# luigifcruz/radio-core

Hardware: AMD Instinct MI355X
Metric: IQ Msamples/s through Tuner+WBFM at 1024 channels (higher is better)
Workload: dtype f32

## Files before the change

### include/rcfm_tools.h

```cpp
#ifndef RCFM_TOOLS_H
#define RCFM_TOOLS_H

#include "rcfm.h"

#ifdef __cplusplus
extern "C" {
#endif

typedef struct rcfm_arena_s* rcfm_arena_t;

int rcfm_arena_create(size_t block_bytes, rcfm_arena_t* out);
int rcfm_arena_adopt(void* base, size_t bytes, rcfm_arena_t* out);
int rcfm_arena_bind(rcfm_arena_t arena);
int rcfm_arena_stats(rcfm_arena_t arena, size_t* reserved_bytes, size_t* used_bytes, size_t* live_pieces);
int rcfm_arena_destroy(rcfm_arena_t arena);


enum { RCFM_TUNER_OPT_NARROW_TILES = 1,
       RCFM_TUNER_OPT_ALIGNED_PLAN = 2 };
int rcfm_tuner_set_option(rcfm_tuner_t t, int option, int value);

enum { RCFM_OPT_LDS_CHAIN = 1, RCFM_OPT_FUSED_TILES = 2, RCFM_OPT_PHASE_LINK = 3, RCFM_OPT_PILOT_CHAIN = 6, RCFM_OPT_DECIM_TILE = 7,
       RCFM_OPT_LDS_DEEMPH = 8, RCFM_OPT_PILOT_BLOCKED = 9, RCFM_OPT_SSB_DIRECT = 11 };
int rcfm_demod_get_option(rcfm_demod_t d, int option, int* value);


typedef struct rcfm_fft_pass {
    int32_t L, nstages, radix[8];
    int64_t n_o1, n_o2, n_inner;
    int64_t in_o1, in_o2, in_i, in_l;
    int64_t out_o1, out_o2, out_i, out_k;
    int64_t tw_o1, tw_o2, tw_i;
    int32_t has_twiddle, load_along_l;
    int64_t in_t, out_t;
    int32_t flat_outer;
    int32_t reserved_;
} rcfm_fft_pass;
typedef struct rcfm_fft_plan {
// ... 23 lines not shown
```

### radio-core_amd/csrc/api_internal.h

```cpp
#pragma once

#include <algorithm>
#include <atomic>
#include <cstdlib>
#include <map>
#include <memory>
#include <mutex>
#include <string>
#include <vector>

#include "common.h"
#include "fft_engine.h"
#include "fft_plan.h"
#include "fused_passes.h"
#include "kernels.h"
#include "lds_chain.h"

#define TILE_CALL(narrow_tiles, fn, ...) ((narrow_tiles) ? ::rcfm::narrow::fn(__VA_ARGS__) : ::rcfm::fn(__VA_ARGS__))

namespace rcfm {

constexpr double kPi = 3.14159265358979323846;


// ... 132 lines not shown
    }();
    return v;
}

inline void require_channels(int first, int count, int n) {
    RC_REQUIRE(first >= 0 && count >= 0 && first + count <= n, RCFM_ERR_INDEX, "channel index out of range");
}

}


struct rcfm_tuner_s {
    rcfm::Arena* arena = rcfm::arena_enter_handle();
    ~rcfm_tuner_s() { rcfm::arena_leave_handle(arena); }
    int opt_narrow = rcfm::kNarrowDefault;
    int64_t n = 0;
    int nch = 0;
    std::vector<int64_t> roll;
    std::vector<int32_t> bw;
    rcfm::DeviceBuffer roll_dev;
    rcfm::DeviceBuffer base_dev;
    rcfm::DeviceBuffer bw_dev;
    rcfm::DeviceBuffer levels_part;
    rcfm::DeviceBuffer power_part_sum, power_part_max;
    rcfm::DeviceBuffer X;
    int64_t halo = 0;
    float2* ext = nullptr;
    bool ext_window = false;
    int ext_first = 0, ext_count = 0;
    float2* spectrum() { return (ext ? ext : X.as<float2>()) + halo; }
// ... 60 lines not shown
```

### radio-core_amd/csrc/demod.hip

```cpp

#include <cmath>
#include <cstring>

#include "api_internal.h"

using namespace rcfm;

struct rcfm_demod_s {
    Arena* arena = arena_enter_handle();
    ~rcfm_demod_s() {
        drop_graphs();
        if (cap_stream) (void)hipStreamDestroy(cap_stream);
        arena_leave_handle(arena);
    }
    int kind = 0, C = 0, B = 0, A = 0, ch = 1, chunk = 1;
    double tau = 75e-6;
    float taps_h[51];
    float zi_h[50];
    float pilot_h[41];
    float pilot_g_h[41];
    DeviceBuffer taps, pilot_g;
    struct StateBuf : DeviceBuffer {
        hipEvent_t ev = nullptr;
        bool armed = false, recorded = false;
// ... 18 lines not shown
    float side_tap = 0.23f;
    ResampleGeom geom;
    PlanCache r2c_B, c2c_inv_B, c2c_fwd_B, c2c_inv_A, c2r_A;
    std::unique_ptr<FftEngine> eng_B, eng_A;
    std::unique_ptr<FftEngine> eng_Ad;
    std::unique_ptr<FftEngine> eng_Bi;
    DeviceBuffer buf_Ti;
    bool opt_lds_chain = true;
    bool opt_pilot_chain = true;
    bool opt_decim_tile = true;
    bool opt_pilot_blocked = true;
    bool opt_phase_link = true;
    bool opt_lds_deemph = true;
    bool opt_ssb_direct = true;
    int opt_narrow = kNarrowDefault;
    bool opt_graph = false;
    struct GraphSlot {
        const void* iq;
        void* audio;
        const float* state;
        int first;
        hipGraphExec_t exec;
        uint64_t used;
    };
    std::vector<GraphSlot> graphs;
    GraphSlot last_call{nullptr, nullptr, nullptr, -1, nullptr, 0};
    hipStream_t cap_stream = nullptr;
    uint64_t graph_tick = 0;
    void drop_graphs() {
        for (auto& g : graphs) (void)hipGraphExecDestroy(g.exec);
// ... 641 lines not shown

int rcfm_demod_set_option(rcfm_demod_t d, int option, int value) {
    return guarded([&] {
        RC_REQUIRE(d, RCFM_ERR_ARG, "NULL handle");
        d->drop_graphs();
        switch (option) {
            case RCFM_OPT_GRAPH: d->opt_graph = value != 0; break;
            case RCFM_OPT_LDS_CHAIN: d->opt_lds_chain = value != 0; break;
            case RCFM_OPT_FUSED_TILES: d->opt_pilot_chain = d->opt_decim_tile = value != 0; break;
            case RCFM_OPT_PILOT_CHAIN: d->opt_pilot_chain = value != 0; break;
            case RCFM_OPT_DECIM_TILE: d->opt_decim_tile = value != 0; break;
            case RCFM_OPT_PILOT_BLOCKED: d->opt_pilot_blocked = value != 0; break;
            case RCFM_OPT_LDS_DEEMPH: d->opt_lds_deemph = value != 0; break;
            case RCFM_OPT_PHASE_LINK: d->opt_phase_link = value != 0; break;
            case RCFM_OPT_SSB_DIRECT: d->opt_ssb_direct = value != 0; break;
            case RCFM_OPT_NARROW_TILES:
                RC_REQUIRE(value >= 0 && value <= 2, RCFM_ERR_ARG, "narrow tiles: 0 never, 1 automatic, 2 always");
                d->opt_narrow = value;
                break;
            case RCFM_OPT_STATE_FENCE: {
                auto& b = *d->state_buf;
                if (value != 0 && b.ev == nullptr) RC_HIP(hipEventCreateWithFlags(&b.ev, hipEventDisableTiming));
                b.armed = value != 0;
                if (!b.armed) b.recorded = false;
                break;
            }
            default: RC_REQUIRE(false, RCFM_ERR_ARG, "unknown demodulator option");
        }
    });
}
// ... 1 lines not shown
int rcfm_demod_get_option(rcfm_demod_t d, int option, int* value) {
    return guarded([&] {
        RC_REQUIRE(d && value, RCFM_ERR_ARG, "NULL handle or output");
        switch (option) {
            case RCFM_OPT_LDS_CHAIN: *value = d->opt_lds_chain; break;
            case RCFM_OPT_FUSED_TILES: *value = d->opt_pilot_chain && d->opt_decim_tile; break;
            case RCFM_OPT_PILOT_CHAIN: *value = d->opt_pilot_chain; break;
            case RCFM_OPT_DECIM_TILE: *value = d->opt_decim_tile; break;
            case RCFM_OPT_PILOT_BLOCKED:
                *value = d->opt_pilot_blocked && d->opt_pilot_chain && d->pilot_blocked().valid() &&
                         fused_pilot_chain_applies(*d->eng_B, *d->eng_Bi, 2);
                break;
            case RCFM_OPT_LDS_DEEMPH: *value = d->opt_lds_deemph; break;
            case RCFM_OPT_PHASE_LINK: *value = d->opt_phase_link; break;
            case RCFM_OPT_SSB_DIRECT: *value = d->opt_ssb_direct; break;
            case RCFM_OPT_NARROW_TILES: *value = d->opt_narrow; break;
            case RCFM_OPT_STATE_FENCE: *value = d->state_buf->armed; break;
            case RCFM_OPT_GRAPH: *value = d->opt_graph ? 1 + (int)d->graphs.size() : 0; break;
            default: RC_REQUIRE(false, RCFM_ERR_ARG, "unknown demodulator option");
        }
    });
}

int rcfm_demod_get_taps(rcfm_demod_t d, float* deemph51_host, float* pilot41_host) {
    return guarded([&] {
        RC_REQUIRE(d, RCFM_ERR_ARG, "NULL handle");
        if (deemph51_host) std::memcpy(deemph51_host, d->taps_h, sizeof(d->taps_h));
        if (pilot41_host) std::memcpy(pilot41_host, d->pilot_h, sizeof(d->pilot_h));
    });
}
// ... 62 lines not shown
```

### radio-core_amd/csrc/fft_engine.h

```cpp
#pragma once

#include <cstdint>

#include "common.h"

namespace rcfm {

constexpr int kFftTileW = 16;
constexpr int kFftMaxStages = 8;
constexpr int kFftMaxPasses = 4;
constexpr int kFftMaxL = 512;
constexpr int kFftBigL = 640;

struct FftPass {
    int L;
    int nstages;
    int radix[kFftMaxStages];
    int64_t n_o1, n_o2, n_inner;
    int64_t in_o1, in_o2, in_i, in_l;
    int64_t out_o1, out_o2, out_i, out_k;
    int64_t tw_o1, tw_o2, tw_i;
    int has_twiddle;
    int load_along_l;
    int64_t in_t, out_t;
// ... 33 lines not shown
   public:
    explicit FftEngine(int64_t n);
    FftEngine(int64_t n, const int64_t* factors, int nfactors, int layout = -1);
    const FftPlanDesc& desc() const { return desc_; }
    bool has_blocked() const { return has_blk_; }
    const FftPlanDesc& desc_blocked() const { return has_blk_ ? desc_blk_ : desc_; }
    int npass() const { return desc_.npass; }
    int64_t tmp_stride() const { return desc_.tmp_stride; }
    void c2c(const float2* in, float2* out, float2* tmp, int batch, bool inverse, float scale,
             hipStream_t stream, const FftRowWindow* keep = nullptr, float2* tmp2 = nullptr) const;
    int64_t row_length() const { return desc_.pass[0].L; }
    FftPassDev pass_dev(int t, int64_t in_batch, int64_t out_batch, bool blocked = false) const;
    static size_t lds_bytes(int L);
    static dim3 grid(const FftPass& p, int batch);
    static int compute_units();

   private:
    void build_tables();
    void split_layouts();
    FftPlanDesc desc_;
    FftPlanDesc desc_blk_;
    bool has_blk_ = false;
    DeviceBuffer stage_tw_[kFftMaxPasses];
    DeviceBuffer pos_[kFftMaxPasses];
    DeviceBuffer coarse_;
};

}
```

### radio-core_amd/csrc/fft_kernel.h

```cpp
#pragma once

#include <hip/hip_runtime.h>

#include <cstdio>
#include <cstdlib>
#include <type_traits>

#include "fft_engine.h"
#include "tile_ns.h"

namespace rcfm {
RCFM_NS_OPEN
namespace fftk {

constexpr int W = RCFM_TILE_W;
constexpr int kLogW = W == 16 ? 4 : W == 8 ? 3 : 2;
static_assert((1 << kLogW) == W, "tile width: 4, 8 or 16 lines");
constexpr int kThreads = 256 * W / 16;

__device__ __forceinline__ float2 cmul(float2 a, float2 b) {
    typedef float v2f __attribute__((ext_vector_type(2)));
    v2f A, B, D;
    A.x = a.x; A.y = a.y; B.x = b.x; B.y = b.y;
    asm("v_pk_mul_f32 %0, %1, %2 op_sel:[0,0] op_sel_hi:[0,1]" : "=v"(D) : "v"(A), "v"(B));
// ... 506 lines not shown
__device__ __forceinline__ int last_stage_base(int g) {
    if constexpr (S == 2) {
        return g;
    } else if constexpr (S == 3) {
        constexpr int w1 = L / (R0 * RL);
        const int q1 = g / w1, q2 = g - q1 * w1;
        return q1 + R0 * q2;
    } else {
        constexpr int w1 = L / (R0 * RL), w2 = L / (R0 * R1 * RL);
        const int q1 = g / w1, r1 = g - q1 * w1;
        const int q2 = r1 / w2, q3 = r1 - q2 * w2;
        return q1 + R0 * (q2 + R1 * q3);
    }
}

template <int L, int R0, int R1, int R2, int R3, bool ROWS, int T, class LoadOp, class StoreOp>
__global__ __launch_bounds__(T, (big_tile_pair(L) ? 8 : triple_tile(L) ? 6 : T * 16 / W >= 512 ? 4 : 1)) void k_fft_tile(FftPassDev d, LoadOp load,
                                                                                          StoreOp store) {
    constexpr bool BIG = big_tile_pair(L) || triple_tile(L);
    constexpr int S = (R0 > 1) + (R1 > 1) + (R2 > 1) + (R3 > 1);
    static_assert(S >= 2 && R0 * R1 * R2 * R3 == L, "bad radix list");
    constexpr int RL = (S == 2) ? R1 : (S == 3) ? R2 : R3;
    constexpr int m0 = L / R0;
    constexpr int RG = T / W;
    constexpr int nit0 = (m0 + RG - 1) / RG;
    constexpr int nld = ROWS ? (L * W + T - 1) / T : nit0 * R0;
    __shared__ __attribute__((aligned(16))) float2 tile[L * (ROWS && !BIG ? kRowsPitch : W)];
    __shared__ __attribute__((aligned(16))) float2 tw_lds[BIG ? 1 : L];
    const float2* tw = BIG ? d.stage_tw : tw_lds;
    const FftPass& p = d.p;

    const int tid = threadIdx.x;
    const int w = tid & (W - 1), rg = tid >> kLogW;
    const VBlock vb = vblock_hw();
    LineId id;
    BlockPos bp = block_pos(vb);
    id.batch = bp.batch;
    unsigned o = vb.y;
    const unsigned n_o2 = (unsigned)p.n_o2;
    if (p.flat_outer) {
        const unsigned tiles_inner = ((unsigned)p.n_inner + W - 1) / W;
        o = bp.tile / tiles_inner;
        if (o >= (unsigned)(p.n_o1 * p.n_o2)) return;
        bp.tile -= o * tiles_inner;
    }
    id.o1 = n_o2 == 1 ? o : o / n_o2;
    id.o2 = n_o2 == 1 ? 0 : o - (unsigned)id.o1 * n_o2;
    const int i0 = (int)bp.tile * W;
    const int left = (int)p.n_inner - i0;
    const int wvalid = left < W ? left : W;
    const int64_t in_base = (int64_t)id.batch * d.in_batch + id.o1 * p.in_o1 + id.o2 * p.in_o2 +
                            (p.in_t ? (int64_t)(i0 >> 4) * p.in_t + (i0 & 15) : (int64_t)i0 * p.in_i);
    const int64_t out_base = (int64_t)id.batch * d.out_batch + id.o1 * p.out_o1 + id.o2 * p.out_o2 +
                             (p.out_t ? (int64_t)(i0 >> 4) * p.out_t + (i0 & 15) : (int64_t)i0);
    const unsigned in_l = (unsigned)p.in_l, in_i = (unsigned)p.in_i, out_k = (unsigned)p.out_k;

    constexpr int NF = fetch_count<LoadOp>::value;
    constexpr bool HZ = !ROWS && has_half_zones<LoadOp>::value && L % 2 == 0;
    auto zone = [](int q) -> int { return (q + 1) * m0 <= L / 2 ? 0 : (q * m0 > L / 2 ? 2 : 1); };
    float2 v[nld];
    float2 v2[NF >= 2 ? nld : 1];
    float v3[NF == 3 ? nld : 1];
    static_assert(NF <= 2 || !ROWS, "three-fetch load functors: strided passes only");
    if constexpr (ROWS) {
#pragma unroll
        for (int it = 0; it < nld; ++it) {
            int e = tid + T * it;
            if ((L * W) % T != 0) e = e < L * W ? e : 0;
            const int wl = e / L, l = e - wl * L;
            const int wc = wl < wvalid ? wl : 0;
            id.i = i0 + wc;
            v[it] = load.fetch(id, l, in_base, (unsigned)wc * in_i + (unsigned)l);
            if constexpr (NF == 2) v2[it] = load.fetch2(id, l, in_base, (unsigned)wc * in_i + (unsigned)l);
        }
    } else {
        const int wc = w < wvalid ? w : 0;
        id.i = i0 + wc;
#pragma unroll
        for (int it = 0; it < nit0; ++it) {
            int b = rg + RG * it;
            if (m0 % RG != 0) b = b < m0 ? b : 0;
#pragma unroll
            for (int q = 0; q < R0; ++q) {
                const int l = b + q * m0;
                if constexpr (HZ) {
                    const int z = zone(q);
                    if (z == 2) {
                        v[it * R0 + q] = make_float2(0.f, 0.f);
                        if constexpr (NF == 2) v2[it * R0 + q] = make_float2(0.f, 0.f);
                    } else {
                        v[it * R0 + q] = load.fetch(id, l, in_base, (unsigned)l * in_l + (unsigned)wc, z);
                        if constexpr (NF == 2)
// ... 24 lines not shown
            return g;
        } else if constexpr (S == 3) {
            constexpr int w1 = L / (R0 * RL);
            const int q1 = g / w1, q2 = g - q1 * w1;
            return q1 + R0 * q2;
        } else {
            constexpr int w1 = L / (R0 * RL), w2 = L / (R0 * R1 * RL);
            const int q1 = g / w1, r1 = g - q1 * w1;
            const int q2 = r1 / w2, q3 = r1 - q2 * w2;
            return q1 + R0 * (q2 + R1 * q3);
        }
    };
    constexpr bool AUX = has_aux<StoreOp>::value;
    float aux[AUX ? nitL * RL : 1];
    if constexpr (AUX) {
        const int wc = w < wvalid ? w : 0;
        id.i = i0 + wc;
#pragma unroll
        for (int it = 0; it < nitL; ++it) {
            int g = rg + RG * it;
            if (rowsL % RG != 0) g = g < rowsL ? g : 0;
            const int kb = kbase(g);
#pragma unroll
            for (int q = 0; q < RL; ++q) {
                const int k = kb + (L / RL) * q;
                aux[it * RL + q] = store.fetch_aux(id, k, out_base, (unsigned)k * out_k + (unsigned)wc);
            }
        }
    }

    if constexpr (ROWS) {
#pragma unroll
        for (int it = 0; it < nld; ++it) {
            const int e = tid + T * it;
            const int wl = e / L, l = e - wl * L;
            id.i = i0 + wl;
            float2 x;
            if constexpr (NF == 2) x = load.post(id, l, v[it], v2[it]);
            else x = load.post(id, l, v[it]);
            if ((L * W) % T == 0 || e < L * W) tile[lds_slot<true, !BIG>(l, wl)] = x;
        }
        __syncthreads();
        stage_lds<L, R0, L, true, RG, !BIG, BIG>(tile, tw, w, rg);
    } else {
        if constexpr (!BIG) __syncthreads();
        id.i = i0 + (w < wvalid ? w : 0);
#pragma unroll
        for (int it = 0; it < nit0; ++it) {
            const int b = rg + RG * it;
            if ((m0 % RG == 0) || b < m0) {
                float2* x = &v[it * R0];
#pragma unroll
                for (int q = 0; q < R0; ++q) {
                    if constexpr (HZ) {
                        if constexpr (NF == 2) {
                            if (zone(q) != 2) x[q] = load.post(id, b + q * m0, x[q], v2[it * R0 + q], zone(q));
                        } else {
                            if (zone(q) != 2) x[q] = load.post(id, b + q * m0, x[q], zone(q));
                        }
                    } else if constexpr (NF == 3) x[q] = load.post(id, b + q * m0, x[q], v2[it * R0 + q], v3[it * R0 + q]);
                    else if constexpr (NF == 2) x[q] = load.post(id, b + q * m0, x[q], v2[it * R0 + q]);
// ... 13 lines not shown
#pragma unroll
                for (int q = 0; q < R0; ++q) tile[lds_slot<false>(b + q * m0, w)] = x[dft_slot<R0>(q)];
            }
        }
    }
    __syncthreads();
    if constexpr (S >= 3) {
        stage_lds<L, R1, L / R0, ROWS, RG, !BIG, BIG>(tile, tw, w, rg);
        __syncthreads();
    }
    if constexpr (S >= 4) {
        stage_lds<L, R2, L / (R0 * R1), ROWS, RG, !BIG, BIG>(tile, tw, w, rg);
        __syncthreads();
    }

    const unsigned f = (unsigned)(id.o1 * p.tw_o1 + id.o2 * p.tw_o2 + (int64_t)(i0 + w) * p.tw_i);
    float2 D = make_float2(1.f, 0.f);
    constexpr bool PTW = !ROWS;
    if constexpr (PTW) D = big_twiddle(d, f * (unsigned)(L / RL));
    id.i = i0 + w;
    const bool lane_ok = w < wvalid;
#pragma unroll
    for (int it = 0; it < nitL; ++it) {
        const int g = rg + RG * it;
        if ((rowsL % RG == 0) || g < rowsL) {
            float2 x[RL];
#pragma unroll
            for (int q = 0; q < RL; ++q) x[q] = tile[lds_slot<ROWS, !BIG>(g * RL + q, w)];
            dft_p<RL>(x);
            const int kb = kbase(g);
            float2 Tw = make_float2(1.f, 0.f);
            if constexpr (PTW) Tw = big_twiddle(d, f * (unsigned)kb);
            if (lane_ok) {
#pragma unroll
                for (int q = 0; q < RL; ++q) {
                    const int k = kb + (L / RL) * q;
                    float2 y = x[dft_slot<RL>(q)];
                    if constexpr (PTW) {
                        y = cmul(y, Tw);
                        Tw = cmul(Tw, D);
                    }
                    if constexpr (AUX) store(id, k, out_base, (unsigned)k * out_k + (unsigned)w, y, aux[it * RL + q]);
                    else store(id, k, out_base, (unsigned)k * out_k + (unsigned)w, y);
                }
            }
        }
    }
}

template <class T, class = void>
struct mid_upper_rows_zero : std::false_type {};
template <class T>
struct mid_upper_rows_zero<T, std::void_t<decltype(T::kUpperRowsZero)>> : std::bool_constant<T::kUpperRowsZero> {};

template <int L, int R0, int R1, int R2, int R3, int T, class LoadOp, class MidOp, class StoreOp>
__global__ __launch_bounds__(T, (T * 16 / W >= 512 ? 4 : 1)) void k_fft_tile2(FftPassDev d1, FftPassDev d2, LoadOp load,
                                                                     MidOp mid, StoreOp store) {
    constexpr int S = (R0 > 1) + (R1 > 1) + (R2 > 1) + (R3 > 1);
    static_assert(S >= 2 && R0 * R1 * R2 * R3 == L, "bad radix list");
    constexpr int RL = (S == 2) ? R1 : (S == 3) ? R2 : R3;
    constexpr int RG = T / W;
    constexpr int nld = (L * W + T - 1) / T;
// ... 579 lines not shown
}

template <class T> struct is_plain_functor : std::false_type {};
template <bool S> struct is_plain_functor<LoadPlainT<S>> : std::true_type {};
template <bool S> struct is_plain_functor<StorePlainT<S>> : std::true_type {};
template <> struct is_plain_functor<StoreRowWindow> : std::true_type {};

enum PassKinds : int { kAnyPass = 0, kStridedOnly = 1, kRowsOnly = 2 };

template <int LEN, int A, int B, int C, int D, bool ROWS, class LoadOp, class StoreOp>
inline void launch_fft_tile_one(const FftPassDev& d, dim3 grid, const LoadOp& ld, const StoreOp& st, hipStream_t s) {
    constexpr int T = tile_threads(LEN);
    hipLaunchKernelGGL((k_fft_tile<LEN, A, B, C, D, ROWS, T, LoadOp, StoreOp>), grid, dim3(T), 0, s, d, ld, st);
}

template <int KIND = kAnyPass, class LoadOp, class StoreOp>
inline void launch_fft_pass(const FftPassDev& d, int batch, const LoadOp& ld, const StoreOp& st, hipStream_t s) {
    bool done = false;
    const bool rows = d.p.load_along_l != 0;
    RC_REQUIRE(!(KIND == kStridedOnly && rows) && !(KIND == kRowsOnly && !rows), RCFM_ERR_RUNTIME,
               "FFT functor used with the wrong pass kind");
    const bool shape_ok = (rows || d.p.in_i == 1) && d.p.out_i == 1 && ((d.p.has_twiddle != 0) == !rows) &&
                          d.p.n_o1 * d.p.n_o2 <= 65535 && batch <= 65535;
    if (shape_ok) {
        const unsigned tiles_inner = (unsigned)((d.p.n_inner + W - 1) / W), outer = (unsigned)(d.p.n_o1 * d.p.n_o2);
        const dim3 grid = d.p.flat_outer ? dim3((tiles_inner * outer + 7u) / 8u * 8u, 1, (unsigned)batch)
                                         : dim3(tiles_inner, outer, (unsigned)batch);
        switch (d.p.L) {
#define RCFM_CASE(LEN, A, B, C, D)                                                                            \
    case LEN:                                                                                                 \
        if (rows) {                                                                                           \
            if constexpr (KIND != kStridedOnly)                                                               \
                launch_fft_tile_one<LEN, A, B, C, D, true, LoadOp, StoreOp>(d, grid, ld, st, s);               \
        } else {                                                                                              \
            if constexpr (KIND != kRowsOnly)                                                                  \
                launch_fft_tile_one<LEN, A, B, C, D, false, LoadOp, StoreOp>(d, grid, ld, st, s);              \
        }                                                                                                     \
        done = true;                                                                                          \
// ... 113 lines not shown
```

### radio-core_amd/csrc/fused_passes.hip

```cpp
#include "fused_passes.h"
#include "device_math.h"

#include "fft_kernel.h"
#include "fft_decim_rt.h"
#include "kernels.h"

namespace rcfm {
RCFM_NS_OPEN

using fftk::LineId;
using fftk::kAnyPass;
using fftk::kRowsOnly;
using fftk::kStridedOnly;

namespace {


struct LoadTunerGatherFast {
    const float2* X;
    const int32_t* base;
    float two_pi_over_n, delta;
    float c0, c1, c2, c3;
    int B, nyq;
    int merge;
// ... 502 lines not shown
    fftk::StorePlainT<true> stl{z, (float)(1.0 / (double)n)};
    fftk::launch_fft_pass<kRowsOnly>(e.pass_dev(np - 1, e.tmp_stride(), n), count, ldl, stl, s);
}
void fused_real_pair_fft(const FftEngine& e, const float* x, float2* U, float2* tmp, int count, int keep,
                         hipStream_t s, bool from_phase, PhaseRows rows) {
    if (count <= 0) return;
    const int64_t n = e.desc().n;
    const int np = e.npass();
    const int pairs = (count + 1) / 2;
    fftk::StorePlainT<false> st0{tmp, 1.0f};
    if (from_phase) {
        const LoadPhaseStepPair ld = phase_pair_load(x, n, count, (int)e.desc().pass[0].in_l, rows);
        fftk::launch_fft_pass<kStridedOnly>(e.pass_dev(0, 0, e.tmp_stride()), pairs, ld, st0, s);
    } else {
        LoadRealPair ld{x, (int)n, count};
        fftk::launch_fft_pass<kStridedOnly>(e.pass_dev(0, 0, e.tmp_stride()), pairs, ld, st0, s);
    }
    middle_passes(e, 1, np - 2, tmp, pairs, s);
    fftk::LoadPlainT<false> ldl{tmp};
    if (keep >= 0 || keep == kKeepLowerHalf) {
        StorePruned stl{U, (int)n, keep};
        fftk::launch_fft_pass<kRowsOnly>(e.pass_dev(np - 1, e.tmp_stride(), n), pairs, ldl, stl, s);
    } else {
        fftk::StorePlainT<false> stl{U, 1.0f};
        fftk::launch_fft_pass<kRowsOnly>(e.pass_dev(np - 1, e.tmp_stride(), n), pairs, ldl, stl, s);
    }
}

void fused_hilbert_pair_ifft_mix(const FftEngine& e, const float2* U, const float* m, float2* u, float2* tmp,
                                 int count, hipStream_t s) {
    if (count <= 0) return;
// ... 75 lines not shown
    const FftPass& p0 = ef.desc().pass[0];
    if (p0.load_along_l || p0.in_i != 1 || p0.n_o1 != 1 || p0.n_o2 != 1 || (int64_t)p0.L * p0.in_l != ef.desc().n ||
        p0.n_inner != p0.in_l)
        return false;
    *rows = p0.L;
    *row_length = p0.in_l;
    return true;
}

void fused_pilot_chain_fft_first(const FftEngine& ef, const float* p, float2* tmp_f, int count, hipStream_t s,
                                 int64_t blk_stride, int blk16) {
    if (count <= 0) return;
    const int64_t n = ef.desc().n;
    LoadRealPair ld{p, (int)n, count, blk_stride, blk16};
    fftk::StorePlainT<false> st0{tmp_f, 1.0f};
    fftk::launch_fft_pass<kStridedOnly>(ef.pass_dev(0, 0, ef.tmp_stride()), (count + 1) / 2, ld, st0, s);
}

void fused_pilot_chain_mask_mix(const FftEngine& ef, const FftEngine& ei, const float* p, const float* m,
                                float2* tmp_f, float2* tmp_i, int count, hipStream_t s, int64_t blk_stride, int blk16) {
    if (count <= 0) return;
    const int64_t n = ef.desc().n;
    const int pairs = (count + 1) / 2;
    {
        const FftPassDev d1 = ef.pass_dev(1, ef.tmp_stride(), n);
        const FftPassDev d2 = ei.pass_dev(0, n, ei.tmp_stride());
        fftk::LoadPlainT<false> ld{tmp_f};
        fftk::StorePlainT<false> st{tmp_i, 1.0f};
        const float scale = (float)(1.0 / (double)n);
        bool ok;
        if (d1.p.L % 2 == 0 && (int64_t)d1.p.L * d1.p.out_k == n)
// ... 45 lines not shown
    WinAudioDecim win{wr, dc, scale, (int)A, ef.desc().pass[0].L, 0};
    fftk::StorePlainT<false> st{tmp_a, 1.0f};
    {
        const FftPassDev d1 = ef.pass_dev(1, ef.tmp_stride(), B), d2 = ea.pass_dev(0, A, ea.tmp_stride());
        RC_REQUIRE(fftk::launch_fft_tile2_decim(d1, d2, count, ld, win, st, s) || decim_rt(d1, d2, count, tmp_f, win, tmp_a, s),
                   RCFM_ERR_RUNTIME, "decimating two-transform kernel refused a pair it should accept");
    }
    fftk::LoadPlainT<false> ldl{tmp_a};
    fftk::StorePlainT<true> stl{out, 1.0f};
    FftPassDev last = ea.pass_dev(1, ea.tmp_stride(), A);
    if (out_pitch > 0) {
        RC_REQUIRE(out_pitch >= last.p.out_k && last.p.n_o1 * last.p.n_o2 == 1, RCFM_ERR_RUNTIME, "bad audio row pitch");
        last.out_batch = (A / last.p.out_k) * (int64_t)out_pitch;
        last.p.out_k = out_pitch;
    }
    fftk::launch_fft_pass<kRowsOnly>(last, count, ldl, stl, s);
}

struct StoreRealImagSplit {
    float* y;
    int n, count;
    __device__ __forceinline__ void operator()(const LineId& id, int, int64_t base, unsigned off, float2 v) const {
        const int64_t t = base + off - (int64_t)id.batch * n;
        const int c0 = 2 * id.batch;
        y[(int64_t)c0 * n + t] = v.y;
        if (c0 + 1 < count) y[(int64_t)(c0 + 1) * n + t] = v.x;
    }
};

void fused_real_pair_fft_first(const FftEngine& e, const float* x, float2* tmp, int count, bool from_phase,
                               hipStream_t s, PhaseRows rows) {
    if (count <= 0) return;
    const int64_t n = e.desc().n;
    const int pairs = (count + 1) / 2;
    fftk::StorePlainT<false> st0{tmp, 1.0f};
    if (from_phase) {
        const LoadPhaseStepPair ld = phase_pair_load(x, n, count, (int)e.desc().pass[0].in_l, rows);
        fftk::launch_fft_pass<kStridedOnly>(e.pass_dev(0, 0, e.tmp_stride()), pairs, ld, st0, s);
    } else {
        LoadRealPair ld{x, (int)n, count};
        fftk::launch_fft_pass<kStridedOnly>(e.pass_dev(0, 0, e.tmp_stride()), pairs, ld, st0, s);
    }
}

void fused_fft_decim_ifft_pairs(const FftEngine& ef, const FftEngine& ea, const float2* tmp_f, float* y,
                                float2* tmp_a, int count, const float* wr, float scale, float2* dc, hipStream_t s) {
    if (count <= 0) return;
    const int64_t B = ef.desc().n, A = ea.desc().n;
    const int pairs = (count + 1) / 2;
    fftk::LoadPlainT<false> ld{tmp_f};
    WinAudioDecim win{wr, dc, scale, (int)A, ef.desc().pass[0].L, count};
    fftk::StorePlainT<false> st{tmp_a, 1.0f};
    {
        const FftPassDev d1 = ef.pass_dev(1, ef.tmp_stride(), B), d2 = ea.pass_dev(0, A, ea.tmp_stride());
        RC_REQUIRE(fftk::launch_fft_tile2_decim(d1, d2, pairs, ld, win, st, s) || decim_rt(d1, d2, pairs, tmp_f, win, tmp_a, s),
                   RCFM_ERR_RUNTIME, "decimating two-transform kernel refused a pair it should accept");
// ... 143 lines not shown
```

### radio-core_amd/csrc/tuner.hip

```cpp

#include "api_internal.h"

using namespace rcfm;

bool rcfm_tuner_s::row_window(int first, int count, FftRowWindow* w, const FftEngine* eng) const {
    if (!eng) eng = forward_engine.get();
    if (!eng || count == 0) return false;
    const int64_t f0 = eng->row_length();
    const int64_t rows = n / f0;
    if (rows < 64) return false;
    std::vector<char> used((size_t)rows, 0);
    for (int c = first; c < first + count; ++c) {
        const int64_t centre = (n - roll[c]) % n, h = bw[c] / 2 + 2;
        const int64_t r0 = (centre - h) / f0 - ((centre - h) < 0 ? 1 : 0), r1 = (centre + h) / f0;
        for (int64_t r = r0; r <= r1; ++r) used[(size_t)(((r % rows) + rows) % rows)] = 1;
    }
    int64_t best_len = 0, best_start = 0, run = 0;
    for (int64_t i = 0; i < 2 * rows; ++i) {
        if (!used[(size_t)(i % rows)]) {
            ++run;
            if (run > best_len && run <= rows) {
                best_len = run;
                best_start = i - run + 1;
            }
// ... 59 lines not shown
    bool ok = halo > 0 && count > 0;
    if (ok) {
        bin_window(first, count, fb, nb);
        ok = *nb < n && *fb >= halo && *fb + *nb <= n - halo;
    }
    RC_REQUIRE(ok, RCFM_ERR_SIZE,
               "these channels' bins wrap around the ends of the spectrum (or are all of it): no window storage");
}

rcfm_tuner_s::Band& rcfm_tuner_s::band(int32_t b) {
    auto it = bands.find(b);
    if (it == bands.end()) {
        auto nb = std::make_unique<Band>();
        nb->geom.build(n, b, 0.5 , true);
        FftPlanDesc probe;
        if (use_engine() && fft_plan_describe(b, &probe)) nb->engine = std::make_unique<FftEngine>(b);
        it = bands.emplace(b, std::move(nb)).first;
    }
    return *it->second;
}

bool rcfm_tuner_s::fast_gather_ok(int first) {
    if (first < 0 || first >= nch || halo <= 0) return false;
    const int32_t B = bw[first];
    const ResampleGeom& g = band(B).geom;
    const bool series = 6.28318530717958647692 * ((double)(B / 2 + 2) / (double)n) < 0.25;
    return series && halo >= B / 2 + 1 && g.nyq_mode != NYQ_UP && B <= n;
}

bool rcfm_tuner_s::fast_bins_ok(int32_t B) const {
    const bool series = 6.28318530717958647692 * ((double)(B / 2 + 2) / (double)n) < 0.25;
// ... 283 lines not shown
        t->ext_first = first;
        t->ext_count = count;
        t->set_loaded(false, false, first, 0);
    });
}

int rcfm_tuner_set_option(rcfm_tuner_t t, int option, int value) {
    return guarded([&] {
        RC_REQUIRE(t, RCFM_ERR_ARG, "NULL handle");
        switch (option) {
            case RCFM_TUNER_OPT_NARROW_TILES:
                RC_REQUIRE(value >= 0 && value <= 2, RCFM_ERR_ARG, "narrow tiles: 0 never, 1 automatic, 2 always");
                t->opt_narrow = value;
                break;
            case RCFM_TUNER_OPT_ALIGNED_PLAN: t->opt_aligned = value != 0; break;
            default: RC_REQUIRE(false, RCFM_ERR_ARG, "unknown tuner option");
        }
    });
}

int rcfm_tuner_window(rcfm_tuner_t t, int first, int count, int64_t* first_bin, int64_t* nbins) {
    return guarded([&] {
        RC_REQUIRE(t && first_bin && nbins, RCFM_ERR_ARG, "NULL argument");
        require_channels(first, count, t->nch);
        t->bin_window(first, count, first_bin, nbins);
    });
}

int rcfm_tuner_adopt(rcfm_tuner_t t, int first, int count, void* stream) {
    return guarded([&] {
// ... 11 lines not shown
```

### radio-core_amd/radiocore/_internal/hip.py

```python

import ctypes
import os
import sys
import threading
import warnings

import numpy as np

_HERE = os.path.dirname(os.path.abspath(__file__))
LIB_PATH = os.environ.get("RCFM_LIB") or os.path.join(os.path.dirname(_HERE), "_lib", "librcfm.so")

RCFM_FM, RCFM_MFM, RCFM_WBFM = 0, 1, 2
RCFM_AM = 3
RCFM_USB, RCFM_LSB = 5, 6
RCFM_SSB_LEVEL = 0.25
RCFM_OPT_LDS_CHAIN, RCFM_OPT_FUSED_TILES, RCFM_OPT_PHASE_LINK, RCFM_OPT_NARROW_TILES, RCFM_OPT_STATE_FENCE = 1, 2, 3, 4, 5
RCFM_OPT_PILOT_CHAIN, RCFM_OPT_DECIM_TILE, RCFM_OPT_LDS_DEEMPH, RCFM_OPT_PILOT_BLOCKED, RCFM_OPT_GRAPH = 6, 7, 8, 9, 10
RCFM_OPT_SSB_DIRECT = 11
RCFM_TUNER_OPT_NARROW_TILES, RCFM_TUNER_OPT_ALIGNED_PLAN = 1, 2

_ERR_SIZE, _ERR_INDEX, _ERR_RUNTIME, _ERR_ARG, _ERR_STATE = -1, -2, -3, -4, -5

_vp = ctypes.c_void_p
_i = ctypes.c_int
_i64 = ctypes.c_int64
_sz = ctypes.c_size_t
_dbl = ctypes.c_double
_fp = ctypes.POINTER(ctypes.c_float)

SIGNATURES = {
    "rcfm_version": [],
    "rcfm_device_count": [ctypes.POINTER(_i)],
    "rcfm_malloc": [ctypes.POINTER(_vp), _sz],
    "rcfm_free": [_vp],
# ... 280 lines not shown
```

Measured before the change: 34550.

## Pack partial FFT tail tiles from several batches into one shared tile block

```diff
diff --git a/include/rcfm_tools.h b/include/rcfm_tools.h
--- a/include/rcfm_tools.h
+++ b/include/rcfm_tools.h
@@ -17,11 +17,12 @@
 
 
 enum { RCFM_TUNER_OPT_NARROW_TILES = 1,
-       RCFM_TUNER_OPT_ALIGNED_PLAN = 2 };
+       RCFM_TUNER_OPT_ALIGNED_PLAN = 2,
+       RCFM_TUNER_OPT_SHARED_TAILS = 3 };
 int rcfm_tuner_set_option(rcfm_tuner_t t, int option, int value);
 
 enum { RCFM_OPT_LDS_CHAIN = 1, RCFM_OPT_FUSED_TILES = 2, RCFM_OPT_PHASE_LINK = 3, RCFM_OPT_PILOT_CHAIN = 6, RCFM_OPT_DECIM_TILE = 7,
-       RCFM_OPT_LDS_DEEMPH = 8, RCFM_OPT_PILOT_BLOCKED = 9, RCFM_OPT_SSB_DIRECT = 11 };
+       RCFM_OPT_LDS_DEEMPH = 8, RCFM_OPT_PILOT_BLOCKED = 9, RCFM_OPT_SSB_DIRECT = 11, RCFM_OPT_SHARED_TAILS = 12 };
 int rcfm_demod_get_option(rcfm_demod_t d, int option, int* value);
 
 
diff --git a/radio-core_amd/csrc/api_internal.h b/radio-core_amd/csrc/api_internal.h
--- a/radio-core_amd/csrc/api_internal.h
+++ b/radio-core_amd/csrc/api_internal.h
@@ -170,6 +170,7 @@
     rcfm::Arena* arena = rcfm::arena_enter_handle();
     ~rcfm_tuner_s() { rcfm::arena_leave_handle(arena); }
     int opt_narrow = rcfm::kNarrowDefault;
+    bool opt_shared_tails = true;
     int64_t n = 0;
     int nch = 0;
     std::vector<int64_t> roll;
diff --git a/radio-core_amd/csrc/demod.hip b/radio-core_amd/csrc/demod.hip
--- a/radio-core_amd/csrc/demod.hip
+++ b/radio-core_amd/csrc/demod.hip
@@ -56,6 +56,7 @@
     bool opt_lds_deemph = true;
     bool opt_ssb_direct = true;
     int opt_narrow = kNarrowDefault;
+    bool opt_shared_tails = true;
     bool opt_graph = false;
     struct GraphSlot {
         const void* iq;
@@ -727,6 +728,11 @@
             case RCFM_OPT_LDS_DEEMPH: d->opt_lds_deemph = value != 0; break;
             case RCFM_OPT_PHASE_LINK: d->opt_phase_link = value != 0; break;
             case RCFM_OPT_SSB_DIRECT: d->opt_ssb_direct = value != 0; break;
+            case RCFM_OPT_SHARED_TAILS:
+                d->opt_shared_tails = value != 0;
+                for (FftEngine* e : {d->eng_B.get(), d->eng_A.get(), d->eng_Ad.get(), d->eng_Bi.get()})
+                    if (e) e->set_share_tails(d->opt_shared_tails);
+                break;
             case RCFM_OPT_NARROW_TILES:
                 RC_REQUIRE(value >= 0 && value <= 2, RCFM_ERR_ARG, "narrow tiles: 0 never, 1 automatic, 2 always");
                 d->opt_narrow = value;
@@ -758,6 +764,7 @@
             case RCFM_OPT_LDS_DEEMPH: *value = d->opt_lds_deemph; break;
             case RCFM_OPT_PHASE_LINK: *value = d->opt_phase_link; break;
             case RCFM_OPT_SSB_DIRECT: *value = d->opt_ssb_direct; break;
+            case RCFM_OPT_SHARED_TAILS: *value = d->opt_shared_tails; break;
             case RCFM_OPT_NARROW_TILES: *value = d->opt_narrow; break;
             case RCFM_OPT_STATE_FENCE: *value = d->state_buf->armed; break;
             case RCFM_OPT_GRAPH: *value = d->opt_graph ? 1 + (int)d->graphs.size() : 0; break;
diff --git a/radio-core_amd/csrc/fft_engine.h b/radio-core_amd/csrc/fft_engine.h
--- a/radio-core_amd/csrc/fft_engine.h
+++ b/radio-core_amd/csrc/fft_engine.h
@@ -71,8 +71,11 @@
     static size_t lds_bytes(int L);
     static dim3 grid(const FftPass& p, int batch);
     static int compute_units();
+    bool share_tails() const { return share_tails_; }
+    void set_share_tails(bool on) { share_tails_ = on; }
 
    private:
+    bool share_tails_ = true;
     void build_tables();
     void split_layouts();
     FftPlanDesc desc_;
diff --git a/radio-core_amd/csrc/fft_kernel.h b/radio-core_amd/csrc/fft_kernel.h
--- a/radio-core_amd/csrc/fft_kernel.h
+++ b/radio-core_amd/csrc/fft_kernel.h
@@ -544,9 +544,9 @@
     }
 }
 
-template <int L, int R0, int R1, int R2, int R3, bool ROWS, int T, class LoadOp, class StoreOp>
-__global__ __launch_bounds__(T, (big_tile_pair(L) ? 8 : triple_tile(L) ? 6 : T * 16 / W >= 512 ? 4 : 1)) void k_fft_tile(FftPassDev d, LoadOp load,
-                                                                                          StoreOp store) {
+template <int L, int R0, int R1, int R2, int R3, bool ROWS, int T, bool SHARED, class LoadOp, class StoreOp>
+__device__ __forceinline__ void fft_tile_body(const FftPassDev& d, const LoadOp& load, const StoreOp& store, float2* tile,
+                                              float2* tw_lds, BlockPos bp, unsigned o, int rs) {
     constexpr bool BIG = big_tile_pair(L) || triple_tile(L);
     constexpr int S = (R0 > 1) + (R1 > 1) + (R2 > 1) + (R3 > 1);
     static_assert(S >= 2 && R0 * R1 * R2 * R3 == L, "bad radix list");
@@ -555,18 +555,13 @@
     constexpr int RG = T / W;
     constexpr int nit0 = (m0 + RG - 1) / RG;
     constexpr int nld = ROWS ? (L * W + T - 1) / T : nit0 * R0;
-    __shared__ __attribute__((aligned(16))) float2 tile[L * (ROWS && !BIG ? kRowsPitch : W)];
-    __shared__ __attribute__((aligned(16))) float2 tw_lds[BIG ? 1 : L];
     const float2* tw = BIG ? d.stage_tw : tw_lds;
     const FftPass& p = d.p;
 
     const int tid = threadIdx.x;
     const int w = tid & (W - 1), rg = tid >> kLogW;
-    const VBlock vb = vblock_hw();
     LineId id;
-    BlockPos bp = block_pos(vb);
     id.batch = bp.batch;
-    unsigned o = vb.y;
     const unsigned n_o2 = (unsigned)p.n_o2;
     if (p.flat_outer) {
         const unsigned tiles_inner = ((unsigned)p.n_inner + W - 1) / W;
@@ -576,9 +571,13 @@
     }
     id.o1 = n_o2 == 1 ? o : o / n_o2;
     id.o2 = n_o2 == 1 ? 0 : o - (unsigned)id.o1 * n_o2;
-    const int i0 = (int)bp.tile * W;
+    const int i0 = SHARED ? (int)p.n_inner - (1 << rs) : (int)bp.tile * W;
     const int left = (int)p.n_inner - i0;
-    const int wvalid = left < W ? left : W;
+    const int wvalid = SHARED ? W : (left < W ? left : W);
+    const int s0 = (int)bp.batch;
+    auto slot_line = [&](int x) -> int { return SHARED ? (x & ((1 << rs) - 1)) : x; };
+    auto slot_in = [&](int x) -> unsigned { return SHARED ? (unsigned)(x >> rs) * (unsigned)d.in_batch : 0u; };
+    auto slot_out = [&](int x) -> unsigned { return SHARED ? (unsigned)(x >> rs) * (unsigned)d.out_batch : 0u; };
     const int64_t in_base = (int64_t)id.batch * d.in_batch + id.o1 * p.in_o1 + id.o2 * p.in_o2 +
                             (p.in_t ? (int64_t)(i0 >> 4) * p.in_t + (i0 & 15) : (int64_t)i0 * p.in_i);
     const int64_t out_base = (int64_t)id.batch * d.out_batch + id.o1 * p.out_o1 + id.o2 * p.out_o2 +
@@ -598,14 +597,16 @@
             int e = tid + T * it;
             if ((L * W) % T != 0) e = e < L * W ? e : 0;
             const int wl = e / L, l = e - wl * L;
-            const int wc = wl < wvalid ? wl : 0;
+            const int wc = SHARED ? slot_line(wl) : (wl < wvalid ? wl : 0);
             id.i = i0 + wc;
-            v[it] = load.fetch(id, l, in_base, (unsigned)wc * in_i + (unsigned)l);
-            if constexpr (NF == 2) v2[it] = load.fetch2(id, l, in_base, (unsigned)wc * in_i + (unsigned)l);
+            if constexpr (SHARED) id.batch = s0 + (wl >> rs);
+            v[it] = load.fetch(id, l, in_base, (unsigned)wc * in_i + (unsigned)l + slot_in(wl));
+            if constexpr (NF == 2) v2[it] = load.fetch2(id, l, in_base, (unsigned)wc * in_i + (unsigned)l + slot_in(wl));
         }
     } else {
-        const int wc = w < wvalid ? w : 0;
-        id.i = i0 + wc;
+        const int wc = SHARED ? slot_line(w) + (int)slot_in(w) : (w < wvalid ? w : 0);
+        id.i = i0 + slot_line(w < wvalid ? w : 0);
+        if constexpr (SHARED) id.batch = s0 + (w >> rs);
 #pragma unroll
         for (int it = 0; it < nit0; ++it) {
             int b = rg + RG * it;
@@ -660,8 +661,9 @@
     constexpr bool AUX = has_aux<StoreOp>::value;
     float aux[AUX ? nitL * RL : 1];
     if constexpr (AUX) {
-        const int wc = w < wvalid ? w : 0;
-        id.i = i0 + wc;
+        const int wc = SHARED ? slot_line(w) + (int)slot_out(w) : (w < wvalid ? w : 0);
+        id.i = i0 + slot_line(w < wvalid ? w : 0);
+        if constexpr (SHARED) id.batch = s0 + (w >> rs);
 #pragma unroll
         for (int it = 0; it < nitL; ++it) {
             int g = rg + RG * it;
@@ -680,7 +682,8 @@
         for (int it = 0; it < nld; ++it) {
             const int e = tid + T * it;
             const int wl = e / L, l = e - wl * L;
-            id.i = i0 + wl;
+            id.i = i0 + slot_line(wl);
+            if constexpr (SHARED) id.batch = s0 + (wl >> rs);
             float2 x;
             if constexpr (NF == 2) x = load.post(id, l, v[it], v2[it]);
             else x = load.post(id, l, v[it]);
@@ -690,7 +693,7 @@
         stage_lds<L, R0, L, true, RG, !BIG, BIG>(tile, tw, w, rg);
     } else {
         if constexpr (!BIG) __syncthreads();
-        id.i = i0 + (w < wvalid ? w : 0);
+        id.i = i0 + slot_line(w < wvalid ? w : 0);
 #pragma unroll
         for (int it = 0; it < nit0; ++it) {
             const int b = rg + RG * it;
@@ -734,11 +737,13 @@
         __syncthreads();
     }
 
-    const unsigned f = (unsigned)(id.o1 * p.tw_o1 + id.o2 * p.tw_o2 + (int64_t)(i0 + w) * p.tw_i);
+    const unsigned f = (unsigned)(id.o1 * p.tw_o1 + id.o2 * p.tw_o2 + (int64_t)(i0 + slot_line(w)) * p.tw_i);
     float2 D = make_float2(1.f, 0.f);
     constexpr bool PTW = !ROWS;
     if constexpr (PTW) D = big_twiddle(d, f * (unsigned)(L / RL));
-    id.i = i0 + w;
+    id.i = i0 + slot_line(w);
+    if constexpr (SHARED) id.batch = s0 + (w >> rs);
+    const unsigned wo = (unsigned)slot_line(w) + slot_out(w);
     const bool lane_ok = w < wvalid;
 #pragma unroll
     for (int it = 0; it < nitL; ++it) {
@@ -760,12 +765,57 @@
                         y = cmul(y, Tw);
                         Tw = cmul(Tw, D);
                     }
-                    if constexpr (AUX) store(id, k, out_base, (unsigned)k * out_k + (unsigned)w, y, aux[it * RL + q]);
-                    else store(id, k, out_base, (unsigned)k * out_k + (unsigned)w, y);
+                    if constexpr (AUX) store(id, k, out_base, (unsigned)k * out_k + wo, y, aux[it * RL + q]);
+                    else store(id, k, out_base, (unsigned)k * out_k + wo, y);
                 }
             }
         }
     }
+}
+
+template <int L, int R0, int R1, int R2, int R3, bool ROWS, int T, class LoadOp, class StoreOp>
+__global__ __launch_bounds__(T, (big_tile_pair(L) ? 8 : triple_tile(L) ? 6 : T * 16 / W >= 512 ? 4 : 1)) void k_fft_tile(FftPassDev d, LoadOp load,
+                                                                                          StoreOp store) {
+    constexpr bool BIG = big_tile_pair(L) || triple_tile(L);
+    __shared__ __attribute__((aligned(16))) float2 tile[L * (ROWS && !BIG ? kRowsPitch : W)];
+    __shared__ __attribute__((aligned(16))) float2 tw_lds[BIG ? 1 : L];
+    const VBlock vb = vblock_hw();
+    fft_tile_body<L, R0, R1, R2, R3, ROWS, T, false>(d, load, store, tile, tw_lds, block_pos(vb), vb.y, 0);
+}
+
+struct TailShare {
+    unsigned groups, full;
+    int rs;
+};
+__device__ __forceinline__ unsigned xcd_run_item(unsigned x, unsigned count) {
+    const unsigned a = x & 7u, base = count >> 3, extra = count & 7u;
+    return base * a + (a < extra ? a : extra) + (x >> 3);
+}
+
+template <int L, int R0, int R1, int R2, int R3, bool ROWS, int T, class LoadOp, class StoreOp>
+__global__ __launch_bounds__(T, (T * 16 / W >= 512 ? 4 : 1)) void k_fft_tile_st(FftPassDev d, LoadOp load, StoreOp store,
+                                                                               TailShare ts) {
+    static_assert(!big_tile_pair(L) && !triple_tile(L), "shared tail tiles: the 16-line tiles with their table in LDS");
+    __shared__ __attribute__((aligned(16))) float2 tile[L * (ROWS ? kRowsPitch : W)];
+    __shared__ __attribute__((aligned(16))) float2 tw_lds[L];
+    const unsigned g = (unsigned)W >> ts.rs, per_group = g * ts.full + 1u;
+    unsigned n = blockIdx.x;
+    const unsigned q = n / per_group;
+    BlockPos bp;
+    if (q < ts.groups) {
+        const unsigned m = xcd_run_item(n - q * per_group, per_group);
+        if (m == per_group - 1u) {
+            fft_tile_body<L, R0, R1, R2, R3, ROWS, T, true>(d, load, store, tile, tw_lds, BlockPos{ts.full, q * g}, 0u, ts.rs);
+            return;
+        }
+        const unsigned row = m / ts.full;
+        bp = BlockPos{m - row * ts.full, q * g + row};
+    } else {
+        n -= ts.groups * per_group;
+        const unsigned row = n / (ts.full + 1u);
+        bp = BlockPos{xcd_run_item(n - row * (ts.full + 1u), ts.full + 1u), ts.groups * g + row};
+    }
+    fft_tile_body<L, R0, R1, R2, R3, ROWS, T, false>(d, load, store, tile, tw_lds, bp, 0u, 0);
 }
 
 template <class T, class = void>
@@ -1375,14 +1425,66 @@
     hipLaunchKernelGGL((k_fft_tile<LEN, A, B, C, D, ROWS, T, LoadOp, StoreOp>), grid, dim3(T), 0, s, d, ld, st);
 }
 
-template <int KIND = kAnyPass, class LoadOp, class StoreOp>
-inline void launch_fft_pass(const FftPassDev& d, int batch, const LoadOp& ld, const StoreOp& st, hipStream_t s) {
+inline bool tail_share_plan(const FftPassDev& d, int batch, TailShare* ts) {
+    const int64_t r = d.p.n_inner % W, full = d.p.n_inner / W;
+    if (W != 16 || r == 0 || W % r != 0 || full == 0 || d.p.n_o1 * d.p.n_o2 != 1 || d.p.flat_outer) return false;
+    const int64_t g = W / r, groups = batch / g;
+    const int64_t reach = (g - 1) * std::max(std::llabs(d.in_batch), std::llabs(d.out_batch)) +
+                          (int64_t)d.p.L * std::max(d.p.in_l, d.p.out_k) + (W + 1) * std::max<int64_t>(d.p.in_i, d.p.L);
+    if (groups == 0 || d.in_batch < 0 || d.out_batch < 0 || reach >= ((int64_t)1 << 31)) return false;
+    const int64_t blocks = groups * (g * full + 1) + (batch - groups * g) * (full + 1);
+    if (blocks >= ((int64_t)1 << 31)) return false;
+    ts->groups = (unsigned)groups;
+    ts->full = (unsigned)full;
+    ts->rs = r == 1 ? 0 : r == 2 ? 1 : r == 4 ? 2 : 3;
+    return true;
+}
+
+template <int LEN, int A, int B, int C, int D, bool ROWS, class LoadOp, class StoreOp>
+inline void launch_fft_tile_st(const FftPassDev& d, int batch, const TailShare& ts, const LoadOp& ld, const StoreOp& st,
+                               hipStream_t s) {
+    constexpr int T = tile_threads(LEN);
+    const unsigned g = (unsigned)W >> ts.rs;
+    const unsigned blocks = ts.groups * (g * ts.full + 1u) + ((unsigned)batch - ts.groups * g) * (ts.full + 1u);
+    hipLaunchKernelGGL((k_fft_tile_st<LEN, A, B, C, D, ROWS, T, LoadOp, StoreOp>), dim3(blocks), dim3(T), 0, s, d, ld, st, ts);
+}
+
+template <int KIND = kAnyPass, bool SHARE = false, class LoadOp, class StoreOp>
+inline void launch_fft_pass(const FftPassDev& d, int batch, const LoadOp& ld, const StoreOp& st, hipStream_t s,
+                            bool share_tails = false) {
     bool done = false;
     const bool rows = d.p.load_along_l != 0;
     RC_REQUIRE(!(KIND == kStridedOnly && rows) && !(KIND == kRowsOnly && !rows), RCFM_ERR_RUNTIME,
                "FFT functor used with the wrong pass kind");
     const bool shape_ok = (rows || d.p.in_i == 1) && d.p.out_i == 1 && ((d.p.has_twiddle != 0) == !rows) &&
                           d.p.n_o1 * d.p.n_o2 <= 65535 && batch <= 65535;
+    if constexpr (SHARE && W == 16) {
+        TailShare ts;
+        if (shape_ok && share_tails && tail_share_plan(d, batch, &ts)) {
+            switch (d.p.L) {
+#define RCFM_CASE(LEN, A, B, C, D)                                                                            \
+    case LEN:                                                                                                 \
+        if constexpr (!big_tile_pair(LEN) && !triple_tile(LEN)) {                                             \
+            if (rows) {                                                                                       \
+                if constexpr (KIND != kStridedOnly)                                                           \
+                    launch_fft_tile_st<LEN, A, B, C, D, true, LoadOp, StoreOp>(d, batch, ts, ld, st, s);       \
+            } else {                                                                                          \
+                if constexpr (KIND != kRowsOnly)                                                              \
+                    launch_fft_tile_st<LEN, A, B, C, D, false, LoadOp, StoreOp>(d, batch, ts, ld, st, s);      \
+            }                                                                                                 \
+            done = true;                                                                                      \
+        }                                                                                                     \
+        break;
+                RCFM_FFT_FAST_LENGTHS(RCFM_CASE)
+#undef RCFM_CASE
+                default: break;
+            }
+            if (done) {
+                RC_HIP(hipGetLastError());
+                return;
+            }
+        }
+    }
     if (shape_ok) {
         const unsigned tiles_inner = (unsigned)((d.p.n_inner + W - 1) / W), outer = (unsigned)(d.p.n_o1 * d.p.n_o2);
         const dim3 grid = d.p.flat_outer ? dim3((tiles_inner * outer + 7u) / 8u * 8u, 1, (unsigned)batch)
diff --git a/radio-core_amd/csrc/fused_passes.hip b/radio-core_amd/csrc/fused_passes.hip
--- a/radio-core_amd/csrc/fused_passes.hip
+++ b/radio-core_amd/csrc/fused_passes.hip
@@ -540,7 +540,7 @@
         fftk::launch_fft_pass<kStridedOnly>(e.pass_dev(0, 0, e.tmp_stride()), pairs, ld, st0, s);
     } else {
         LoadRealPair ld{x, (int)n, count};
-        fftk::launch_fft_pass<kStridedOnly>(e.pass_dev(0, 0, e.tmp_stride()), pairs, ld, st0, s);
+        fftk::launch_fft_pass<kStridedOnly, true>(e.pass_dev(0, 0, e.tmp_stride()), pairs, ld, st0, s, e.share_tails());
     }
     middle_passes(e, 1, np - 2, tmp, pairs, s);
     fftk::LoadPlainT<false> ldl{tmp};
@@ -646,7 +646,7 @@
     const int64_t n = ef.desc().n;
     LoadRealPair ld{p, (int)n, count, blk_stride, blk16};
     fftk::StorePlainT<false> st0{tmp_f, 1.0f};
-    fftk::launch_fft_pass<kStridedOnly>(ef.pass_dev(0, 0, ef.tmp_stride()), (count + 1) / 2, ld, st0, s);
+    fftk::launch_fft_pass<kStridedOnly, true>(ef.pass_dev(0, 0, ef.tmp_stride()), (count + 1) / 2, ld, st0, s, ef.share_tails());
 }
 
 void fused_pilot_chain_mask_mix(const FftEngine& ef, const FftEngine& ei, const float* p, const float* m,
@@ -722,7 +722,7 @@
         last.out_batch = (A / last.p.out_k) * (int64_t)out_pitch;
         last.p.out_k = out_pitch;
     }
-    fftk::launch_fft_pass<kRowsOnly>(last, count, ldl, stl, s);
+    fftk::launch_fft_pass<kRowsOnly, true>(last, count, ldl, stl, s, ea.share_tails());
 }
 
 struct StoreRealImagSplit {
@@ -747,7 +747,7 @@
         fftk::launch_fft_pass<kStridedOnly>(e.pass_dev(0, 0, e.tmp_stride()), pairs, ld, st0, s);
     } else {
         LoadRealPair ld{x, (int)n, count};
-        fftk::launch_fft_pass<kStridedOnly>(e.pass_dev(0, 0, e.tmp_stride()), pairs, ld, st0, s);
+        fftk::launch_fft_pass<kStridedOnly, true>(e.pass_dev(0, 0, e.tmp_stride()), pairs, ld, st0, s, e.share_tails());
     }
 }
 
diff --git a/radio-core_amd/csrc/tuner.hip b/radio-core_amd/csrc/tuner.hip
--- a/radio-core_amd/csrc/tuner.hip
+++ b/radio-core_amd/csrc/tuner.hip
@@ -97,7 +97,10 @@
         auto nb = std::make_unique<Band>();
         nb->geom.build(n, b, 0.5 , true);
         FftPlanDesc probe;
-        if (use_engine() && fft_plan_describe(b, &probe)) nb->engine = std::make_unique<FftEngine>(b);
+        if (use_engine() && fft_plan_describe(b, &probe)) {
+            nb->engine = std::make_unique<FftEngine>(b);
+            nb->engine->set_share_tails(opt_shared_tails);
+        }
         it = bands.emplace(b, std::move(nb)).first;
     }
     return *it->second;
@@ -411,6 +414,11 @@
                 t->opt_narrow = value;
                 break;
             case RCFM_TUNER_OPT_ALIGNED_PLAN: t->opt_aligned = value != 0; break;
+            case RCFM_TUNER_OPT_SHARED_TAILS:
+                t->opt_shared_tails = value != 0;
+                for (auto& b : t->bands)
+                    if (b.second->engine) b.second->engine->set_share_tails(t->opt_shared_tails);
+                break;
             default: RC_REQUIRE(false, RCFM_ERR_ARG, "unknown tuner option");
         }
     });
diff --git a/radio-core_amd/radiocore/_internal/hip.py b/radio-core_amd/radiocore/_internal/hip.py
--- a/radio-core_amd/radiocore/_internal/hip.py
+++ b/radio-core_amd/radiocore/_internal/hip.py
@@ -16,8 +16,8 @@
 RCFM_SSB_LEVEL = 0.25
 RCFM_OPT_LDS_CHAIN, RCFM_OPT_FUSED_TILES, RCFM_OPT_PHASE_LINK, RCFM_OPT_NARROW_TILES, RCFM_OPT_STATE_FENCE = 1, 2, 3, 4, 5
 RCFM_OPT_PILOT_CHAIN, RCFM_OPT_DECIM_TILE, RCFM_OPT_LDS_DEEMPH, RCFM_OPT_PILOT_BLOCKED, RCFM_OPT_GRAPH = 6, 7, 8, 9, 10
-RCFM_OPT_SSB_DIRECT = 11
-RCFM_TUNER_OPT_NARROW_TILES, RCFM_TUNER_OPT_ALIGNED_PLAN = 1, 2
+RCFM_OPT_SSB_DIRECT, RCFM_OPT_SHARED_TAILS = 11, 12
+RCFM_TUNER_OPT_NARROW_TILES, RCFM_TUNER_OPT_ALIGNED_PLAN, RCFM_TUNER_OPT_SHARED_TAILS = 1, 2, 3
 
 _ERR_SIZE, _ERR_INDEX, _ERR_RUNTIME, _ERR_ARG, _ERR_STATE = -1, -2, -3, -4, -5
 
```

Result: no change. 34580, median of 3 (+0.1%).
